# sanweiliti/RoHM

Hardware: NVIDIA H100
Metric: denoised motion clips/sec (145-frame, 1000-step PoseNet p_sample_loop) (higher is better)
Workload: dtype f32 (fp16 hi/lo error-compensated tensor-core GEMMs)

## Files before the change

### rohm_b200/csrc/graph.cu

```cuda
#include <algorithm>

#include "graph.cuh"

namespace rohm {

cudaError_t KernelPatch::apply(cudaGraphExec_t exec, cudaGraphNode_t node, const cudaKernelNodeParams& captured) const {
  void* args[kMaxArgs];
  std::copy(captured.kernelParams, captured.kernelParams + nargs_, args);
  for (int i = 0; i < n_; ++i) args[slots_[i].index] = const_cast<unsigned char*>(slots_[i].bytes);
  cudaKernelNodeParams kp = captured;
  kp.kernelParams = args;
  return cudaGraphExecKernelNodeSetParams(exec, node, &kp);
}

ForwardGraphs::~ForwardGraphs() {
  if (capture_stream_) cudaStreamDestroy(capture_stream_);
}

int ForwardGraphs::run(rohm_ctx* ctx, int B, int T, StepKind step, bool eager, cudaStream_t st,
                       const std::function<int(cudaStream_t)>& launches, const std::vector<KernelPatch>& patches,
                       const std::vector<int>& lengths) {
  cudaStreamCaptureStatus cap = cudaStreamCaptureStatusNone;
  ROHM_CUDA(ctx, cudaStreamIsCapturing(st, &cap));
  if (eager || !enabled || cap != cudaStreamCaptureStatusNone) return launches(st);

  Entry* g = nullptr;
  for (Entry& e : graphs_)
// ... 55 lines not shown
```

### rohm_b200/csrc/graph.cuh

```cuda
#pragma once
#include <cstring>
#include <functional>
#include <memory>
#include <tuple>
#include <type_traits>
#include <vector>

#include "common.h"

namespace rohm {

template <size_t I, typename V>
struct Arg {
  V value;
};
template <size_t I, typename V>
Arg<I, V> arg(V value) {
  return {value};
}

class KernelPatch {
 public:
  template <typename... P, size_t... I, typename... V>
  KernelPatch(void (*kernel)(P...), Arg<I, V>... args)
// ... 12 lines not shown
  };
  template <typename T, typename V>
  void put(size_t index, const V& value) {
    static_assert(std::is_same<V, T>::value || (std::is_pointer<V>::value && std::is_convertible<V, T>::value),
                  "KernelPatch: the value's type is not the kernel parameter's");
    static_assert(sizeof(T) <= sizeof(Slot::bytes), "KernelPatch: parameter wider than a slot");
    const T v = value;
    slots_[n_].index = index;
    std::memcpy(slots_[n_].bytes, &v, sizeof v);
    ++n_;
  }
  const void* func_;
  int nargs_;
  Slot slots_[kMaxPatched];
  int n_ = 0;
};

enum StepKind : int { kNoStep = 0, kStepSingleStream = 1, kStepPerClip = 2 };

class ForwardGraphs {
 public:
  static constexpr size_t kMaxGraphs = 8;
  bool enabled = true;

  ForwardGraphs() = default;
  ForwardGraphs(const ForwardGraphs&) = delete;
  ForwardGraphs& operator=(const ForwardGraphs&) = delete;
  ~ForwardGraphs();

  int run(rohm_ctx* ctx, int B, int T, StepKind step, bool eager, cudaStream_t st,
// ... 64 lines not shown
```

### rohm_b200/csrc/posenet.cu

```cuda
#include <cmath>
#include <cstdlib>
#include <cstring>
#include <new>

#include "attention.cuh"
#include "common.h"
#include "gemm.cuh"
#include "graph.cuh"
#include "ptx.cuh"

namespace rohm {
namespace {


__device__ __forceinline__ void clip_rows(const int* clip_off, int b, int S, int T, int64_t& row0, int& frames) {
  if (clip_off != nullptr) {
    row0 = clip_off[b];
    frames = clip_off[b + 1] - clip_off[b] - 1;
  } else {
    row0 = static_cast<int64_t>(b) * S;
    frames = T;
  }
}

// ... 176 lines not shown
      l.x = y.x - h.x, l.y = y.y - h.y, l.z = y.z - h.z, l.w = y.w - h.w;
      oh[lane + 32 * i] = h;
      ol[lane + 32 * i] = l;
    }
  }
}

}

struct PoseNetLayerDev {
  PackedWeight qkv, proj, ff1, ff2;
  float *qkv_b, *proj_b, *ff1_b, *ff2_b, *n1_w, *n1_b, *n2_w, *n2_b;
  float *qkv_c = nullptr, *qkv_d = nullptr, *ff1_c = nullptr, *ff1_d = nullptr;
};

}

using namespace rohm;

struct rohm_posenet {
  rohm_ctx* ctx = nullptr;
  DevicePool pool;
  int D = 0, F = 0, L = 0, H = 0, C = 0, Cout = 0, traj = 0, pe_len = 0, passes = 3;
  int kind = kKindTf32;
  int max_batch = 0, max_frames = 0;
  int64_t max_rows = 0;
  int Kin_p = 0;
  PackedWeight w_in, w_cond, w_out;
  float *in_b = nullptr, *cond_b = nullptr, *out_b = nullptr, *pe = nullptr;
  float* time_table = nullptr;
// ... 1 lines not shown
  float *Ain_h = nullptr, *Ain_l = nullptr;
  float *X = nullptr, *Xh = nullptr, *Xl = nullptr, *Y = nullptr, *QKV = nullptr, *CTXh = nullptr, *CTXl = nullptr;
  float *Hh = nullptr, *Hl = nullptr, *condpe = nullptr, *OUT = nullptr;
  float* cond_traj = nullptr;
  int cond_B = -1, cond_T = -1;
  std::vector<int> lengths;
  std::vector<int> cond_lengths;
  int* clip_off = nullptr;
  int* clip_ids = nullptr;
  int packed_rows = 0, n_short = 0, short_tokens = 0, long_tokens = 0;
  int launches = 0;
  ForwardGraphs graphs;
  bool use_pdl = true;
  bool tc_attention = false;
  bool attn_maps = false;
  AttnWgmmaMaps attn_wg{};
  AttnArgs attn{};
  bool fused_ln = false;
  float2* stats1 = nullptr;
  float2* stats2 = nullptr;
  float *out_c = nullptr, *out_d = nullptr;
  bool profiling = false;
  std::vector<cudaEvent_t> prof_events;
  std::vector<int> prof_cat;
  GemmParams g_in{}, g_cond{}, g_out{};
  std::vector<GemmParams> g_qkv, g_proj, g_ff1, g_ff2;
};

enum ProfCat { kCatGemm = 0, kCatAttention = 1, kCatLayerNorm = 2, kCatOther = 3, kNumCats = 4 };

static void prof_begin(rohm_posenet* pn, int cat, cudaStream_t st) {
  if (!pn->profiling) return;
  cudaEvent_t a, b;
  cudaEventCreate(&a);
  cudaEventCreate(&b);
  pn->prof_events.push_back(a);
  pn->prof_events.push_back(b);
  pn->prof_cat.push_back(cat);
  cudaEventRecord(a, st);
}
static void prof_end(rohm_posenet* pn, cudaStream_t st) {
// ... 144 lines not shown
  const int f16 = pn->kind == kKindF16 ? 1 : 0;
  const bool pdl = pn->use_pdl && !pn->profiling;
  switch (pn->D) {
    case 128: launch_ln<128>(in, res, g, b, out, oh, ol, rows, st, f16, pdl); break;
    case 256: launch_ln<256>(in, res, g, b, out, oh, ol, rows, st, f16, pdl); break;
    case 512: launch_ln<512>(in, res, g, b, out, oh, ol, rows, st, f16, pdl); break;
    case 1024: launch_ln<1024>(in, res, g, b, out, oh, ol, rows, st, f16, pdl); break;
    default: return fail(pn->ctx, ROHM_ERR_INVALID, "unsupported d_model %d for LayerNorm", pn->D);
  }
  prof_end(pn, st);
  ROHM_CUDA(pn->ctx, cudaGetLastError());
  pn->launches++;
  return ROHM_OK;
}

static int run_attention(rohm_posenet* pn, int B, int S, cudaStream_t st) {
  if (!pn->lengths.empty()) {
    const int n_long = B - pn->n_short;
    for (int k = 0; k < 2; ++k) {
      AttnArgs a = pn->attn;
      a.clip_off = pn->clip_off;
      a.clip_ids = pn->clip_ids + (k == 0 ? 0 : pn->n_short);
      a.B = k == 0 ? pn->n_short : n_long;
      a.S = k == 0 ? pn->short_tokens : pn->long_tokens;
      if (a.B == 0) continue;
      prof_begin(pn, kCatAttention, st);
      const cudaError_t e = launch_attention(a, k == 0 ? kAttnWgmma : kAttnWgmmaStream, &pn->attn_wg, st,
                                             pn->use_pdl && !pn->profiling);
      prof_end(pn, st);
      ROHM_CUDA(pn->ctx, e);
      pn->launches++;
    }
    return ROHM_OK;
  }
  AttnArgs a = pn->attn;
  a.B = B, a.S = S;
  const bool maps = pn->attn_maps && (pn->tc_attention || S > kAttnWgmmaMaxTokens);
  prof_begin(pn, kCatAttention, st);
  const cudaError_t e = launch_attention(a, kAttnAuto, maps ? &pn->attn_wg : nullptr, st, pn->use_pdl && !pn->profiling);
  prof_end(pn, st);
  ROHM_CUDA(pn->ctx, e);
  pn->launches++;
  return ROHM_OK;
}

static int build_time_table(rohm_posenet* pn, const rohm_posenet_weights* w) {
  const int D = pn->D, R = pn->pe_len;
  const int64_t n = static_cast<int64_t>(R) * D;
  pn->time_table = pn->pool.floats(n);
  if (pn->time_table == nullptr) return fail(pn->ctx, ROHM_ERR_CUDA, "time table alloc failed");
  DevicePool tmp;
  PackedWeight w0, w2;
  float* pe_h = tmp.floats(n);
  float* pe_l = tmp.floats(n);
// ... 9 lines not shown
  ROHM_CUDA(pn->ctx, cudaGetLastError());
  GemmParams g1{}, g2{};
  if ((rc = setup_linear(pn, &g1, pe_h, pe_l, R, D, D, w0, w->t0_b)) != ROHM_OK) return rc;
  g1.act = kActSilu;
  g1.out_hi = h_h, g1.out_lo = h_l, g1.lds = D;
  g1.M = R;
  ROHM_CUDA(pn->ctx, launch_gemm(g1, R, D, w0.block_n, 3, 0));
  if ((rc = setup_linear(pn, &g2, h_h, h_l, R, D, D, w2, bias2)) != ROHM_OK) return rc;
  g2.out = pn->time_table, g2.ldo = D;
  g2.M = R;
  ROHM_CUDA(pn->ctx, launch_gemm(g2, R, D, w2.block_n, 3, 0));
  ROHM_CUDA(pn->ctx, cudaDeviceSynchronize());
  return ROHM_OK;
}

extern "C" int rohm_posenet_create(rohm_ctx* ctx, const rohm_posenet_weights* w, int max_batch, int max_frames,
                                   int precision, rohm_posenet** out) {
  if (ctx == nullptr) return ROHM_ERR_INVALID;
  rohm::DeviceGuard device_guard__(ctx);
  if (w == nullptr || out == nullptr || max_batch <= 0 || max_frames <= 0)
    return fail(ctx, ROHM_ERR_INVALID, "rohm_posenet_create: bad arguments");
  if (precision != ROHM_PRECISION_TF32X3 && precision != ROHM_PRECISION_TF32 && precision != ROHM_PRECISION_F16X2)
    return fail(ctx, ROHM_ERR_INVALID, "rohm_posenet_create: precision must be 3 (TF32x3), 2 (F16x2) or 1 (TF32)");
  if (w->d_model % 128 != 0 || w->d_model % w->num_heads != 0 || w->ff_size % 64 != 0)
    return fail(ctx, ROHM_ERR_INVALID, "rohm_posenet_create: d_model must be a multiple of 128, ff_size of 64");
  const int dh = w->d_model / w->num_heads;
  if (dh != 64 && dh != 128) return fail(ctx, ROHM_ERR_INVALID, "rohm_posenet_create: head dim must be 64 or 128");
  if (max_frames + 1 > w->pe_len)
    return fail(ctx, ROHM_ERR_INVALID, "rohm_posenet_create: %d frames need %d rows of the positional table, which has %d",
                max_frames, max_frames + 1, w->pe_len);
// ... 106 lines not shown
  pn->clip_off = static_cast<int*>(pn->pool.bytes(static_cast<int64_t>(max_batch + 1) * sizeof(int)));
  pn->clip_ids = static_cast<int*>(pn->pool.bytes(static_cast<int64_t>(max_batch) * sizeof(int)));
  if (pn->clip_off == nullptr || pn->clip_ids == nullptr) {
    const int rc = fail(ctx, ROHM_ERR_CUDA, "clip table alloc failed: %s", cudaGetErrorString(pn->pool.last_error()));
    delete pn;
    return rc;
  }

  TRY(setup_linear(pn, &pn->g_in, pn->Ain_h, pn->Ain_l, R, pn->C, pn->Kin_p, pn->w_in, pn->in_b));
  pn->g_in.residual = pn->condpe, pn->g_in.ldr = D;
  pn->g_in.out = pn->X, pn->g_in.ldo = D;
  pn->g_in.out_hi = pn->Xh, pn->g_in.out_lo = pn->Xl, pn->g_in.lds = D;
  TRY(setup_linear(pn, &pn->g_cond, pn->Ain_h, pn->Ain_l, R, pn->C, pn->Kin_p, pn->w_cond, pn->cond_b));
  pn->g_cond.residual = pn->condpe, pn->g_cond.ldr = D;
  pn->g_cond.out = pn->condpe, pn->g_cond.ldo = D;
  TRY(setup_linear(pn, &pn->g_out, pn->Xh, pn->Xl, R, D, D, pn->w_out, pn->out_b));
  pn->g_out.out = pn->OUT, pn->g_out.ldo = pn->Cout;
  if (pn->fused_ln && pn->L > 0)
    pn->g_out.a_stats = pn->stats2, pn->g_out.a_corr = pn->out_c, pn->g_out.bias = pn->out_d, pn->g_out.ln_eps = 1e-5f;
  pn->g_qkv.resize(pn->L), pn->g_proj.resize(pn->L), pn->g_ff1.resize(pn->L), pn->g_ff2.resize(pn->L);
  for (int l = 0; l < pn->L; ++l) {
    PoseNetLayerDev& d = pn->layers[l];
    TRY(setup_linear(pn, &pn->g_qkv[l], pn->Xh, pn->Xl, R, D, D, d.qkv, d.qkv_b));
    if (pn->kind == kKindF16) {
      pn->g_qkv[l].out_hi = pn->QKV;
      pn->g_qkv[l].out_lo = reinterpret_cast<__half*>(pn->QKV) + R * 3 * D;
      pn->g_qkv[l].lds = 3 * D;
    } else {
      pn->g_qkv[l].out = pn->QKV, pn->g_qkv[l].ldo = 3 * D;
    }
    TRY(setup_linear(pn, &pn->g_proj[l], pn->CTXh, pn->CTXl, R, D, D, d.proj, d.proj_b));
    pn->g_proj[l].out = pn->Y, pn->g_proj[l].ldo = D;
    auto producer = [&](GemmParams& g, float2* stats_out, const float2* res_stats, const float* res_gamma, const float* res_beta) {
      g.out = nullptr, g.ldo = 0;
      g.out_hi = pn->Xh, g.out_lo = pn->Xl, g.lds = D;
      g.stats_out = stats_out, g.res_stats = res_stats, g.res_gamma = res_gamma, g.res_beta = res_beta, g.ln_eps = 1e-5f;
    };
    auto consumer = [&](GemmParams& g, const float2* a_stats, const float* c, const float* dvec) {
      g.a_stats = a_stats, g.a_corr = c, g.bias = dvec, g.ln_eps = 1e-5f;
    };
    if (pn->fused_ln) {
      if (l > 0) consumer(pn->g_qkv[l], pn->stats2, d.qkv_c, d.qkv_d);
      producer(pn->g_proj[l], pn->stats1, l > 0 ? pn->stats2 : nullptr, l > 0 ? pn->layers[l - 1].n2_w : nullptr,
               l > 0 ? pn->layers[l - 1].n2_b : nullptr);
    }
    TRY(setup_linear(pn, &pn->g_ff1[l], pn->Xh, pn->Xl, R, D, D, d.ff1, d.ff1_b));
    pn->g_ff1[l].act = kActGelu;
    pn->g_ff1[l].out_hi = pn->Hh, pn->g_ff1[l].out_lo = pn->Hl, pn->g_ff1[l].lds = F;
    TRY(setup_linear(pn, &pn->g_ff2[l], pn->Hh, pn->Hl, R, F, F, d.ff2, d.ff2_b));
    pn->g_ff2[l].out = pn->Y, pn->g_ff2[l].ldo = D;
    if (pn->fused_ln) {
      consumer(pn->g_ff1[l], pn->stats1, d.ff1_c, d.ff1_d);
      producer(pn->g_ff2[l], pn->stats2, pn->stats1, d.n1_w, d.n1_b);
    }
    for (GemmParams* g : {&pn->g_qkv[l], &pn->g_proj[l], &pn->g_ff1[l], &pn->g_ff2[l]}) {
      if (gemm_enable_tma_store(g, R, pn->kind) != 0) {
        const int rc__ = fail(ctx, ROHM_ERR_CUDA, "cuTensorMapEncodeTiled (store map) failed");
        delete pn;
        return rc__;
      }
    }
  }
  if (gemm_enable_tma_store(&pn->g_out, R, pn->kind) != 0) {
    const int rc__ = fail(ctx, ROHM_ERR_CUDA, "cuTensorMapEncodeTiled (store map) failed");
    delete pn;
    return rc__;
  }
#undef TRY

  {
    cudaError_t ea = gemm_init_attributes();
    if (ea == cudaSuccess) ea = attention_init_attributes(max_frames + 1, dh);
    if (ea != cudaSuccess) {
      delete pn;
      return fail(ctx, ROHM_ERR_CUDA, "kernel attribute setup failed: %s", cudaGetErrorString(ea));
    }
  }
  pn->attn.qkv_hi = pn->QKV;
  pn->attn.qkv_lo = reinterpret_cast<const __half*>(pn->QKV) + R * 3 * D;
  pn->attn.rows = R;
  pn->attn.ctx_hi = pn->CTXh, pn->attn.ctx_lo = pn->CTXl;
  pn->attn.D = D, pn->attn.H = pn->H;
  pn->attn.scale = 1.0f / sqrtf(static_cast<float>(dh));
  pn->attn.kind = pn->kind;
  pn->attn_maps = pn->kind == kKindF16 && dh == 128;
  if (pn->attn_maps) {
    const int rcm = attention_wgmma_maps(&pn->attn_wg, pn->attn);
    if (rcm != 0) {
      delete pn;
      return fail(ctx, ROHM_ERR_CUDA, "cuTensorMapEncodeTiled (attention tiles) failed (%d)", rcm);
    }
  }
  const cudaError_t e = cudaDeviceSynchronize();
  if (e != cudaSuccess) {
    delete pn;
    return fail(ctx, ROHM_ERR_CUDA, "weight packing failed: %s", cudaGetErrorString(e));
  }
  *out = pn;
  return ROHM_OK;
}

extern "C" void rohm_posenet_destroy(rohm_posenet* pn) { delete pn; }

extern "C" int rohm_posenet_launches_per_forward(const rohm_posenet* pn) { return pn ? pn->launches : 0; }

static int check_lengths(rohm_posenet* pn, int B, int T, const char* fn) {
// ... 72 lines not shown
      const bool is_short = S <= kAttnWgmmaMaxTokens;
      if (is_short != (pass == 0)) continue;
      ids.push_back(b);
      if (is_short) ++n_short, short_tokens = S > short_tokens ? S : short_tokens;
      else long_tokens = S > long_tokens ? S : long_tokens;
    }
  ROHM_CUDA(ctx, cudaDeviceSynchronize());
  ROHM_CUDA(ctx, cudaMemcpy(pn->clip_off, off.data(), (B + 1) * sizeof(int), cudaMemcpyHostToDevice));
  ROHM_CUDA(ctx, cudaMemcpy(pn->clip_ids, ids.data(), B * sizeof(int), cudaMemcpyHostToDevice));
  pn->lengths = std::move(v);
  pn->packed_rows = off[B];
  pn->n_short = n_short, pn->short_tokens = short_tokens, pn->long_tokens = long_tokens;
  return ROHM_OK;
}

static int forward_launches(rohm_posenet* pn, const float* x_t, const int64_t* timesteps, float* out, int B, int T,
                            cudaStream_t st) {
  rohm_ctx* ctx = pn->ctx;
  rohm::DeviceGuard device_guard__(ctx);
  const int S = T + 1, D = pn->D;
  const bool packed = !pn->lengths.empty();
  const int* off = packed ? pn->clip_off : nullptr;
  const int rows = packed ? pn->packed_rows : B * S;
  pn->launches = 0;
  int rc;

  dim3 grid((T + 31) / 32, (pn->C + 31) / 32, B);
  prof_begin(pn, kCatOther, st);
  const bool pdl = pn->use_pdl && !pn->profiling;
  ROHM_CUDA(ctx, launch_chain(pack_tokens_kernel, grid, dim3(32, 8), 0, st, pdl, x_t, pn->Ain_h, pn->Ain_l, pn->C, T, S, pn->Kin_p,
                              pn->kind == kKindF16 ? 1 : 0, off));
  prof_end(pn, st);
  ROHM_CUDA(ctx, cudaGetLastError());
  pn->launches++;
  if ((rc = run_gemm(pn, pn->g_in, pn->w_in, rows, st)) != ROHM_OK) return rc;
  prof_begin(pn, kCatOther, st);
  ROHM_CUDA(ctx, launch_chain(time_token_gather_kernel, dim3(B), dim3(128), 0, st, pdl, timesteps, pn->time_table, pn->pe_len,
                              pn->X, pn->Xh, pn->Xl, S, D, pn->kind == kKindF16 ? 1 : 0, off));
  prof_end(pn, st);
  ROHM_CUDA(ctx, cudaGetLastError());
  pn->launches++;

  for (int l = 0; l < pn->L; ++l) {
    PoseNetLayerDev& d = pn->layers[l];
    if ((rc = run_gemm(pn, pn->g_qkv[l], d.qkv, rows, st)) != ROHM_OK) return rc;
    if ((rc = run_attention(pn, B, S, st)) != ROHM_OK) return rc;
    if ((rc = run_gemm(pn, pn->g_proj[l], d.proj, rows, st)) != ROHM_OK) return rc;
    if (!pn->fused_ln && (rc = run_ln(pn, pn->Y, pn->X, d.n1_w, d.n1_b, pn->X, pn->Xh, pn->Xl, rows, st)) != ROHM_OK) return rc;
    if ((rc = run_gemm(pn, pn->g_ff1[l], d.ff1, rows, st)) != ROHM_OK) return rc;
    if ((rc = run_gemm(pn, pn->g_ff2[l], d.ff2, rows, st)) != ROHM_OK) return rc;
    if (!pn->fused_ln && (rc = run_ln(pn, pn->Y, pn->X, d.n2_w, d.n2_b, pn->X, pn->Xh, pn->Xl, rows, st)) != ROHM_OK) return rc;
  }
  if ((rc = run_gemm(pn, pn->g_out, pn->w_out, rows, st)) != ROHM_OK) return rc;
  dim3 grid_o((T + 31) / 32, (pn->Cout + 31) / 32, B);
  prof_begin(pn, kCatOther, st);
  ROHM_CUDA(ctx, launch_chain(unpack_tokens_kernel, grid_o, dim3(32, 8), 0, st, pdl, pn->OUT, pn->cond_traj, out, pn->C, pn->Cout,
                              pn->traj, T, S, pn->Cout, off));
  prof_end(pn, st);
  ROHM_CUDA(ctx, cudaGetLastError());
  pn->launches++;
  return ROHM_OK;
}

extern "C" int rohm_posenet_forward(rohm_posenet* pn, const float* x_t, const int64_t* timesteps, float* out, int B,
                                    int T, void* stream);

extern "C" int rohm_posenet_profile(rohm_posenet* pn, const float* x_t, const int64_t* timesteps, float* out, int B,
                                    int T, void* stream, float* ms_by_category, int* launches_by_category) {
  if (pn == nullptr) return ROHM_ERR_INVALID;
  if (ms_by_category == nullptr || launches_by_category == nullptr)
    return fail(pn->ctx, ROHM_ERR_INVALID, "rohm_posenet_profile: null output");
  pn->profiling = true;
  pn->prof_events.clear();
  pn->prof_cat.clear();
  int rc = rohm_posenet_forward(pn, x_t, timesteps, out, B, T, stream);
  pn->profiling = false;
  cudaError_t e = cudaStreamSynchronize(static_cast<cudaStream_t>(stream));
  for (int c = 0; c < kNumCats; ++c) ms_by_category[c] = 0.0f, launches_by_category[c] = 0;
  for (size_t i = 0; i < pn->prof_cat.size(); ++i) {
    float ms = 0.0f;
    if (rc == ROHM_OK && e == cudaSuccess) cudaEventElapsedTime(&ms, pn->prof_events[2 * i], pn->prof_events[2 * i + 1]);
    ms_by_category[pn->prof_cat[i]] += ms;
    launches_by_category[pn->prof_cat[i]]++;
  }
  for (cudaEvent_t ev : pn->prof_events) cudaEventDestroy(ev);
  pn->prof_events.clear();
  pn->prof_cat.clear();
  if (rc != ROHM_OK) return rc;
  ROHM_CUDA(pn->ctx, e);
  return ROHM_OK;
}
// ... 59 lines not shown
  if (rc != ROHM_OK) return rc;
  return forward_or_step(pn, x_t, timesteps, x0_out, B, T, stream, nullptr, &step);
}

extern "C" int rohm_posenet_set_option(rohm_posenet* pn, int option, int value) {
  if (pn == nullptr) return ROHM_ERR_INVALID;
  if (option == 0) {
    pn->graphs.enabled = value != 0;
    return ROHM_OK;
  }
  if (option == 1) {
    if (pn->use_pdl != (value != 0)) pn->graphs.clear();
    pn->use_pdl = value != 0;
    return ROHM_OK;
  }
  return fail(pn->ctx, ROHM_ERR_INVALID, "rohm_posenet_set_option: unknown option %d", option);
}
```

### rohm_b200/csrc/trajnet.cu

```cuda
#include <cmath>
#include <memory>
#include <new>
#include <string>

#include "common.h"
#include "gemm.cuh"
#include "graph.cuh"
#include "groupnorm.cuh"
#include "ptx.cuh"

namespace rohm {
namespace {

__device__ __forceinline__ int packed_frames(const int* clip_off, int b, int T, int Tp) {
  return clip_off[b + 1] - clip_off[b] - (Tp - T);
}

template <bool kPacked>
__global__ void pack_rows_kernel(const float* __restrict__ x, float* __restrict__ hi, float* __restrict__ lo, int T,
                                 int Tp, int C, int ld, int64_t total, int f16, const int* __restrict__ clip_off) {
  const int64_t i = static_cast<int64_t>(blockIdx.x) * blockDim.x + threadIdx.x;
  if (i >= total) return;
  const int c = static_cast<int>(i % C);
  const int64_t bt = i / C;
// ... 217 lines not shown
  Conv cond_down[3];
  Rtb enc[4], mid_block[2], dec[4];
  Conv down[4], up_even[4], up_odd[4];
  Conv final_c, final_o;
  GroupNorm final_gn;
  Act f1;
  struct {
    Conv z0, zero[4], down[4], zero_mid;
    Rtb enc[4], mid_block[2];
  } ctl;
  Act scratchY[2], scratchRes[2], scratchA[2];
  float* scratchSplit[2] = {nullptr, nullptr};
  bool use_splitk = true;
  bool parallel = true;
  cudaStream_t side[3] = {nullptr, nullptr, nullptr};
  std::vector<cudaEvent_t> events;
  size_t ev_next = 0;
  int cond_B = -1;
  int launches = 0;
  ForwardGraphs graphs;
  std::vector<int> lengths;
  std::vector<int> cond_lengths;
  int* clip_off[kLevels] = {};
  unsigned char* row_mask[kLevels] = {};
  int packed_rows[kLevels] = {};
  bool use_pdl = true;
  size_t gn_budget = 0;
  size_t gn_smem_max = 0;
  bool batch_invariant = false;
  ~rohm_trajnet() {
    for (cudaStream_t q : side)
      if (q) cudaStreamDestroy(q);
    for (cudaEvent_t e : events) cudaEventDestroy(e);
  }
};

#define TRY(expr)                     \
  do {                                \
    const int rc__ = (expr);          \
    if (rc__ != ROHM_OK) return rc__; \
  } while (0)

namespace {

int64_t rows_of(const rohm_trajnet* tn, int level) { return static_cast<int64_t>(tn->max_batch) * tn->Tp[level]; }

constexpr int64_t kInvariantPlanRows = 64 * (144 + 32);

// ... 246 lines not shown
  if (tn->batch_invariant && !tn->lengths.empty() && cv.gn_cluster > 1) {
    size_t smem = 0;
    for (int len : tn->lengths) {
      const int Tc = len >> level;
      smem = std::max(smem, gn_slice_bytes(Tc, C, kGroups, gn_pick_cluster(Tc, C, kGroups, kGnClipBudget)));
    }
    ROHM_CUDA(tn->ctx, launch_gn_mish_clip_slices(a, B, cv.gn_cluster, smem, st, tn->use_pdl, tn->clip_off[level]));
  } else {
    ROHM_CUDA(tn->ctx, launch_gn_mish(a, B, cv.gn_cluster, st, tn->use_pdl,
                                      tn->lengths.empty() ? nullptr : tn->clip_off[level]));
  }
  tn->launches++;
  return ROHM_OK;
}

int order_after(rohm_trajnet* tn, cudaStream_t from, cudaStream_t to) {
  if (from == to) return ROHM_OK;
  if (tn->ev_next == tn->events.size()) {
    cudaEvent_t e = nullptr;
    ROHM_CUDA(tn->ctx, cudaEventCreateWithFlags(&e, cudaEventDisableTiming));
    tn->events.push_back(e);
  }
  cudaEvent_t e = tn->events[tn->ev_next++];
  ROHM_CUDA(tn->ctx, cudaEventRecord(e, from));
  ROHM_CUDA(tn->ctx, cudaStreamWaitEvent(to, e, 0));
  return ROHM_OK;
}

int run_rtb(rohm_trajnet* tn, Rtb& r, int B, cudaStream_t st, cudaStream_t side) {
  if (r.has_res) {
    TRY(order_after(tn, st, side));
    TRY(run_conv(tn, r.res, B, side));
  }
  TRY(run_conv(tn, r.c1, B, st));
  const float* tp = r.tp_off >= 0 ? tn->tp + r.tp_off : nullptr;
  TRY(run_gn(tn, r.c1, r.gn[0], B, tp, nullptr, nullptr, r.a1, st));
  TRY(run_conv(tn, r.c2, B, st));
  if (r.has_res) TRY(order_after(tn, side, st));
  return run_gn(tn, r.c2, r.gn[1], B, nullptr, r.residual, r.extra, r.out, st);
}

int trajnet_create(rohm_ctx* ctx, int n_params, const char* const* names, const float* const* ptrs, const int64_t* numels,
                   int time_dim, int cond_dim, int traj_feat_dim, int mid_dim, int trajcontrol, int control_cond_dim,
                   int max_batch, int frames, int precision, bool batch_invariant, rohm_trajnet** out) {
  if (ctx == nullptr) return ROHM_ERR_INVALID;
  rohm::DeviceGuard device_guard__(ctx);
  if (names == nullptr || ptrs == nullptr || numels == nullptr || out == nullptr || max_batch <= 0)
    return fail(ctx, ROHM_ERR_INVALID, "rohm_trajnet_create: bad arguments");
  if (frames <= 0 || frames % 16 != 0)
    return fail(ctx, ROHM_ERR_INVALID, "rohm_trajnet_create: frames (%d) must be a positive multiple of 16 (four "
                "stride-2 stages)", frames);
  if (mid_dim <= 0 || mid_dim % 256 != 0 || time_dim % 2 != 0 || time_dim > 64)
    return fail(ctx, ROHM_ERR_INVALID, "rohm_trajnet_create: mid_dim (%d) must be a positive multiple of 256 (the GroupNorm "
// ... 270 lines not shown
  return ROHM_OK;
}

static int trajnet_forward_launches(rohm_trajnet* tn, const float* x_t, const int64_t* time, float* out, int B,
                                    cudaStream_t st) {
  rohm_ctx* ctx = tn->ctx;
  rohm::DeviceGuard device_guard__(ctx);
  tn->launches = 0;
  TRY(trajnet_pack(tn, x_t, tn->xin, B, st));
  const int td = tn->time_dim;
  trajnet_time_kernel<<<dim3(B, 8), 256, sizeof(float) * 6 * td, st>>>(time, td, tn->w1, tn->b1, tn->w3, tn->b3, tn->wcat, tn->bcat,
                                                            tn->tp_total, tn->tp, tn->time_table, kTimeTableRows);
  ROHM_CUDA(ctx, cudaGetLastError());
  tn->launches++;

  tn->ev_next = 0;
  if (tn->parallel)
    for (cudaStream_t& q : tn->side)
      if (q == nullptr) ROHM_CUDA(ctx, cudaStreamCreateWithFlags(&q, cudaStreamNonBlocking));
  cudaStream_t sC = (tn->parallel && tn->control) ? tn->side[0] : st;
  cudaStream_t r0 = tn->parallel ? tn->side[1] : st;
  cudaStream_t r1 = tn->parallel ? tn->side[2] : sC;
  if (tn->control) {
    auto& ctl = tn->ctl;
    TRY(order_after(tn, st, sC));
    for (int l = 0; l < 4; ++l) {
      TRY(run_rtb(tn, ctl.enc[l], B, sC, r1));
      TRY(run_conv(tn, ctl.zero[l], B, sC));
      TRY(run_conv(tn, ctl.down[l], B, sC));
    }
    for (Rtb& r : ctl.mid_block) TRY(run_rtb(tn, r, B, sC, r1));
    TRY(run_conv(tn, ctl.zero_mid, B, sC));
  }

  for (int l = 0; l < 4; ++l) {
    TRY(run_rtb(tn, tn->enc[l], B, st, r0));
    TRY(run_conv(tn, tn->down[l], B, st));
  }
  TRY(run_rtb(tn, tn->mid_block[0], B, st, r0));
  if (tn->control) TRY(order_after(tn, sC, st));
  TRY(run_rtb(tn, tn->mid_block[1], B, st, r0));
  for (int l = 3; l >= 0; --l) {
    TRY(order_after(tn, st, r0));
    TRY(run_conv(tn, tn->up_odd[l], B, r0));
    TRY(run_conv(tn, tn->up_even[l], B, st));
    TRY(order_after(tn, r0, st));
    TRY(run_rtb(tn, tn->dec[l], B, st, r0));
  }
  TRY(run_conv(tn, tn->final_c, B, st));
  TRY(run_gn(tn, tn->final_c, tn->final_gn, B, nullptr, nullptr, nullptr, tn->f1, st));
  TRY(run_conv(tn, tn->final_o, B, st));
  const Act& o = tn->final_o.out;
  const int64_t total = static_cast<int64_t>(B) * tn->T * o.C;
  const bool packed = !tn->lengths.empty();
  (packed ? unpack_rows_kernel<true> : unpack_rows_kernel<false>)<<<static_cast<unsigned>((total + 255) / 256), 256, 0, st>>>(
      o.f32, out, tn->T, tn->Tp[0], o.C, o.ld, total, packed ? tn->clip_off[0] : nullptr);
  ROHM_CUDA(ctx, cudaGetLastError());
  tn->launches++;
  return ROHM_OK;
}

// ... 77 lines not shown
```

Before: 20.16.

## Split PoseNet batch into two clip groups run on parallel streams

When the QKV GEMM tile count exceeds the SM count, the batch is split at a tile-aligned clip boundary into two row groups. Each group gets its own GEMM and attention parameter chain and runs on its own stream, forked and joined with events, so one group's attention and layer-norm phases can overlap the other group's GEMMs. The event-ordering helper moves out of TrajNet into a shared BranchEvents class. The cost is a second stream, extra per-shape plans and tensor maps, and smaller GEMMs that may use tensor cores less efficiently.

```diff
diff --git a/rohm_b200/csrc/graph.cu b/rohm_b200/csrc/graph.cu
--- a/rohm_b200/csrc/graph.cu
+++ b/rohm_b200/csrc/graph.cu
@@ -11,6 +11,23 @@
   cudaKernelNodeParams kp = captured;
   kp.kernelParams = args;
   return cudaGraphExecKernelNodeSetParams(exec, node, &kp);
+}
+
+BranchEvents::~BranchEvents() {
+  for (cudaEvent_t e : events_) cudaEventDestroy(e);
+}
+
+int BranchEvents::order_after(rohm_ctx* ctx, cudaStream_t from, cudaStream_t to) {
+  if (from == to) return ROHM_OK;
+  if (next_ == events_.size()) {
+    cudaEvent_t e = nullptr;
+    ROHM_CUDA(ctx, cudaEventCreateWithFlags(&e, cudaEventDisableTiming));
+    events_.push_back(e);
+  }
+  cudaEvent_t e = events_[next_++];
+  ROHM_CUDA(ctx, cudaEventRecord(e, from));
+  ROHM_CUDA(ctx, cudaStreamWaitEvent(to, e, 0));
+  return ROHM_OK;
 }
 
 ForwardGraphs::~ForwardGraphs() {
diff --git a/rohm_b200/csrc/graph.cuh b/rohm_b200/csrc/graph.cuh
--- a/rohm_b200/csrc/graph.cuh
+++ b/rohm_b200/csrc/graph.cuh
@@ -50,6 +50,20 @@
   int nargs_;
   Slot slots_[kMaxPatched];
   int n_ = 0;
+};
+
+class BranchEvents {
+ public:
+  BranchEvents() = default;
+  BranchEvents(const BranchEvents&) = delete;
+  BranchEvents& operator=(const BranchEvents&) = delete;
+  ~BranchEvents();
+  void rewind() { next_ = 0; }
+  int order_after(rohm_ctx* ctx, cudaStream_t from, cudaStream_t to);
+
+ private:
+  std::vector<cudaEvent_t> events_;
+  size_t next_ = 0;
 };
 
 enum StepKind : int { kNoStep = 0, kStepSingleStream = 1, kStepPerClip = 2 };
diff --git a/rohm_b200/csrc/posenet.cu b/rohm_b200/csrc/posenet.cu
--- a/rohm_b200/csrc/posenet.cu
+++ b/rohm_b200/csrc/posenet.cu
@@ -1,6 +1,7 @@
 #include <cmath>
 #include <cstdlib>
 #include <cstring>
+#include <memory>
 #include <new>
 
 #include "attention.cuh"
@@ -214,6 +215,19 @@
   float *qkv_c = nullptr, *qkv_d = nullptr, *ff1_c = nullptr, *ff1_d = nullptr;
 };
 
+struct LayerChain {
+  int64_t row0 = 0, rows = 0;
+  std::vector<GemmParams> qkv, proj, ff1, ff2;
+  GemmParams out{};
+  AttnArgs attn{};
+  AttnWgmmaMaps attn_wg{};
+};
+
+struct GroupPlan {
+  int B = 0, T = 0, split = 0;
+  LayerChain chain[2];
+};
+
 }
 
 using namespace rohm;
@@ -245,8 +259,6 @@
   bool use_pdl = true;
   bool tc_attention = false;
   bool attn_maps = false;
-  AttnWgmmaMaps attn_wg{};
-  AttnArgs attn{};
   bool fused_ln = false;
   float2* stats1 = nullptr;
   float2* stats2 = nullptr;
@@ -254,8 +266,16 @@
   bool profiling = false;
   std::vector<cudaEvent_t> prof_events;
   std::vector<int> prof_cat;
-  GemmParams g_in{}, g_cond{}, g_out{};
-  std::vector<GemmParams> g_qkv, g_proj, g_ff1, g_ff2;
+  GemmParams g_in{}, g_cond{};
+  LayerChain whole;
+  std::vector<std::unique_ptr<GroupPlan>> plans;
+  cudaStream_t side = nullptr;
+  BranchEvents forks;
+  int num_sms = 0;
+  int groups = 0;
+  ~rohm_posenet() {
+    if (side) cudaStreamDestroy(side);
+  }
 };
 
 enum ProfCat { kCatGemm = 0, kCatAttention = 1, kCatLayerNorm = 2, kCatOther = 3, kNumCats = 4 };
@@ -430,18 +450,18 @@
   return ROHM_OK;
 }
 
-static int run_attention(rohm_posenet* pn, int B, int S, cudaStream_t st) {
+static int run_attention(rohm_posenet* pn, const LayerChain& c, int B, int S, cudaStream_t st) {
   if (!pn->lengths.empty()) {
     const int n_long = B - pn->n_short;
     for (int k = 0; k < 2; ++k) {
-      AttnArgs a = pn->attn;
+      AttnArgs a = c.attn;
       a.clip_off = pn->clip_off;
       a.clip_ids = pn->clip_ids + (k == 0 ? 0 : pn->n_short);
       a.B = k == 0 ? pn->n_short : n_long;
       a.S = k == 0 ? pn->short_tokens : pn->long_tokens;
       if (a.B == 0) continue;
       prof_begin(pn, kCatAttention, st);
-      const cudaError_t e = launch_attention(a, k == 0 ? kAttnWgmma : kAttnWgmmaStream, &pn->attn_wg, st,
+      const cudaError_t e = launch_attention(a, k == 0 ? kAttnWgmma : kAttnWgmmaStream, &c.attn_wg, st,
                                              pn->use_pdl && !pn->profiling);
       prof_end(pn, st);
       ROHM_CUDA(pn->ctx, e);
@@ -449,11 +469,11 @@
     }
     return ROHM_OK;
   }
-  AttnArgs a = pn->attn;
+  AttnArgs a = c.attn;
   a.B = B, a.S = S;
   const bool maps = pn->attn_maps && (pn->tc_attention || S > kAttnWgmmaMaxTokens);
   prof_begin(pn, kCatAttention, st);
-  const cudaError_t e = launch_attention(a, kAttnAuto, maps ? &pn->attn_wg : nullptr, st, pn->use_pdl && !pn->profiling);
+  const cudaError_t e = launch_attention(a, kAttnAuto, maps ? &c.attn_wg : nullptr, st, pn->use_pdl && !pn->profiling);
   prof_end(pn, st);
   ROHM_CUDA(pn->ctx, e);
   pn->launches++;
@@ -493,6 +513,71 @@
   return ROHM_OK;
 }
 
+static int build_chain(rohm_posenet* pn, int64_t row0, int64_t rows, LayerChain* c) {
+  const int D = pn->D, F = pn->F, eb = gemm_elem_bytes(pn->kind);
+  const int64_t R = pn->max_rows;
+  auto at = [&](void* base, int64_t ld, int bytes) { return reinterpret_cast<float*>(static_cast<char*>(base) + row0 * ld * bytes); };
+  float *Xh = at(pn->Xh, D, eb), *Xl = at(pn->Xl, D, eb), *CTXh = at(pn->CTXh, D, eb), *CTXl = at(pn->CTXl, D, eb);
+  float *Hh = at(pn->Hh, F, eb), *Hl = at(pn->Hl, F, eb), *Y = at(pn->Y, D, 4), *OUT = at(pn->OUT, pn->Cout, 4);
+  float* qkv_hi = at(pn->QKV, 3 * D, eb);
+  float* qkv_lo = at(reinterpret_cast<__half*>(pn->QKV) + R * 3 * D, 3 * D, eb);
+  float2* stats1 = pn->fused_ln ? pn->stats1 + row0 * 8 : nullptr;
+  float2* stats2 = pn->fused_ln ? pn->stats2 + row0 * 8 : nullptr;
+  c->row0 = row0, c->rows = rows;
+  int rc;
+  if ((rc = setup_linear(pn, &c->out, Xh, Xl, rows, D, D, pn->w_out, pn->out_b)) != ROHM_OK) return rc;
+  c->out.out = OUT, c->out.ldo = pn->Cout;
+  if (pn->fused_ln && pn->L > 0)
+    c->out.a_stats = stats2, c->out.a_corr = pn->out_c, c->out.bias = pn->out_d, c->out.ln_eps = 1e-5f;
+  c->qkv.resize(pn->L), c->proj.resize(pn->L), c->ff1.resize(pn->L), c->ff2.resize(pn->L);
+  for (int l = 0; l < pn->L; ++l) {
+    PoseNetLayerDev& d = pn->layers[l];
+    if ((rc = setup_linear(pn, &c->qkv[l], Xh, Xl, rows, D, D, d.qkv, d.qkv_b)) != ROHM_OK) return rc;
+    if (pn->kind == kKindF16) {
+      c->qkv[l].out_hi = qkv_hi, c->qkv[l].out_lo = qkv_lo, c->qkv[l].lds = 3 * D;
+    } else {
+      c->qkv[l].out = qkv_hi, c->qkv[l].ldo = 3 * D;
+    }
+    if ((rc = setup_linear(pn, &c->proj[l], CTXh, CTXl, rows, D, D, d.proj, d.proj_b)) != ROHM_OK) return rc;
+    c->proj[l].out = Y, c->proj[l].ldo = D;
+    auto producer = [&](GemmParams& g, float2* stats_out, const float2* res_stats, const float* res_gamma, const float* res_beta) {
+      g.out = nullptr, g.ldo = 0;
+      g.out_hi = Xh, g.out_lo = Xl, g.lds = D;
+      g.stats_out = stats_out, g.res_stats = res_stats, g.res_gamma = res_gamma, g.res_beta = res_beta, g.ln_eps = 1e-5f;
+    };
+    auto consumer = [&](GemmParams& g, const float2* a_stats, const float* cv, const float* dvec) {
+      g.a_stats = a_stats, g.a_corr = cv, g.bias = dvec, g.ln_eps = 1e-5f;
+    };
+    if (pn->fused_ln) {
+      if (l > 0) consumer(c->qkv[l], stats2, d.qkv_c, d.qkv_d);
+      producer(c->proj[l], stats1, l > 0 ? stats2 : nullptr, l > 0 ? pn->layers[l - 1].n2_w : nullptr,
+               l > 0 ? pn->layers[l - 1].n2_b : nullptr);
+    }
+    if ((rc = setup_linear(pn, &c->ff1[l], Xh, Xl, rows, D, D, d.ff1, d.ff1_b)) != ROHM_OK) return rc;
+    c->ff1[l].act = kActGelu;
+    c->ff1[l].out_hi = Hh, c->ff1[l].out_lo = Hl, c->ff1[l].lds = F;
+    if ((rc = setup_linear(pn, &c->ff2[l], Hh, Hl, rows, F, F, d.ff2, d.ff2_b)) != ROHM_OK) return rc;
+    c->ff2[l].out = Y, c->ff2[l].ldo = D;
+    if (pn->fused_ln) {
+      consumer(c->ff1[l], stats1, d.ff1_c, d.ff1_d);
+      producer(c->ff2[l], stats2, stats1, d.n1_w, d.n1_b);
+    }
+    for (GemmParams* g : {&c->qkv[l], &c->proj[l], &c->ff1[l], &c->ff2[l]})
+      if (gemm_enable_tma_store(g, rows, pn->kind) != 0) return fail(pn->ctx, ROHM_ERR_CUDA, "cuTensorMapEncodeTiled (store map) failed");
+  }
+  if (gemm_enable_tma_store(&c->out, rows, pn->kind) != 0)
+    return fail(pn->ctx, ROHM_ERR_CUDA, "cuTensorMapEncodeTiled (store map) failed");
+  AttnArgs& a = c->attn;
+  a.qkv_hi = qkv_hi, a.qkv_lo = qkv_lo, a.rows = rows;
+  a.ctx_hi = CTXh, a.ctx_lo = CTXl;
+  a.D = D, a.H = pn->H;
+  a.scale = 1.0f / sqrtf(static_cast<float>(D / pn->H));
+  a.kind = pn->kind;
+  if (pn->attn_maps && (rc = attention_wgmma_maps(&c->attn_wg, a)) != 0)
+    return fail(pn->ctx, ROHM_ERR_CUDA, "cuTensorMapEncodeTiled (attention tiles) failed (%d)", rc);
+  return ROHM_OK;
+}
+
 extern "C" int rohm_posenet_create(rohm_ctx* ctx, const rohm_posenet_weights* w, int max_batch, int max_frames,
                                    int precision, rohm_posenet** out) {
   if (ctx == nullptr) return ROHM_ERR_INVALID;
@@ -629,60 +714,6 @@
   TRY(setup_linear(pn, &pn->g_cond, pn->Ain_h, pn->Ain_l, R, pn->C, pn->Kin_p, pn->w_cond, pn->cond_b));
   pn->g_cond.residual = pn->condpe, pn->g_cond.ldr = D;
   pn->g_cond.out = pn->condpe, pn->g_cond.ldo = D;
-  TRY(setup_linear(pn, &pn->g_out, pn->Xh, pn->Xl, R, D, D, pn->w_out, pn->out_b));
-  pn->g_out.out = pn->OUT, pn->g_out.ldo = pn->Cout;
-  if (pn->fused_ln && pn->L > 0)
-    pn->g_out.a_stats = pn->stats2, pn->g_out.a_corr = pn->out_c, pn->g_out.bias = pn->out_d, pn->g_out.ln_eps = 1e-5f;
-  pn->g_qkv.resize(pn->L), pn->g_proj.resize(pn->L), pn->g_ff1.resize(pn->L), pn->g_ff2.resize(pn->L);
-  for (int l = 0; l < pn->L; ++l) {
-    PoseNetLayerDev& d = pn->layers[l];
-    TRY(setup_linear(pn, &pn->g_qkv[l], pn->Xh, pn->Xl, R, D, D, d.qkv, d.qkv_b));
-    if (pn->kind == kKindF16) {
-      pn->g_qkv[l].out_hi = pn->QKV;
-      pn->g_qkv[l].out_lo = reinterpret_cast<__half*>(pn->QKV) + R * 3 * D;
-      pn->g_qkv[l].lds = 3 * D;
-    } else {
-      pn->g_qkv[l].out = pn->QKV, pn->g_qkv[l].ldo = 3 * D;
-    }
-    TRY(setup_linear(pn, &pn->g_proj[l], pn->CTXh, pn->CTXl, R, D, D, d.proj, d.proj_b));
-    pn->g_proj[l].out = pn->Y, pn->g_proj[l].ldo = D;
-    auto producer = [&](GemmParams& g, float2* stats_out, const float2* res_stats, const float* res_gamma, const float* res_beta) {
-      g.out = nullptr, g.ldo = 0;
-      g.out_hi = pn->Xh, g.out_lo = pn->Xl, g.lds = D;
-      g.stats_out = stats_out, g.res_stats = res_stats, g.res_gamma = res_gamma, g.res_beta = res_beta, g.ln_eps = 1e-5f;
-    };
-    auto consumer = [&](GemmParams& g, const float2* a_stats, const float* c, const float* dvec) {
-      g.a_stats = a_stats, g.a_corr = c, g.bias = dvec, g.ln_eps = 1e-5f;
-    };
-    if (pn->fused_ln) {
-      if (l > 0) consumer(pn->g_qkv[l], pn->stats2, d.qkv_c, d.qkv_d);
-      producer(pn->g_proj[l], pn->stats1, l > 0 ? pn->stats2 : nullptr, l > 0 ? pn->layers[l - 1].n2_w : nullptr,
-               l > 0 ? pn->layers[l - 1].n2_b : nullptr);
-    }
-    TRY(setup_linear(pn, &pn->g_ff1[l], pn->Xh, pn->Xl, R, D, D, d.ff1, d.ff1_b));
-    pn->g_ff1[l].act = kActGelu;
-    pn->g_ff1[l].out_hi = pn->Hh, pn->g_ff1[l].out_lo = pn->Hl, pn->g_ff1[l].lds = F;
-    TRY(setup_linear(pn, &pn->g_ff2[l], pn->Hh, pn->Hl, R, F, F, d.ff2, d.ff2_b));
-    pn->g_ff2[l].out = pn->Y, pn->g_ff2[l].ldo = D;
-    if (pn->fused_ln) {
-      consumer(pn->g_ff1[l], pn->stats1, d.ff1_c, d.ff1_d);
-      producer(pn->g_ff2[l], pn->stats2, pn->stats1, d.n1_w, d.n1_b);
-    }
-    for (GemmParams* g : {&pn->g_qkv[l], &pn->g_proj[l], &pn->g_ff1[l], &pn->g_ff2[l]}) {
-      if (gemm_enable_tma_store(g, R, pn->kind) != 0) {
-        const int rc__ = fail(ctx, ROHM_ERR_CUDA, "cuTensorMapEncodeTiled (store map) failed");
-        delete pn;
-        return rc__;
-      }
-    }
-  }
-  if (gemm_enable_tma_store(&pn->g_out, R, pn->kind) != 0) {
-    const int rc__ = fail(ctx, ROHM_ERR_CUDA, "cuTensorMapEncodeTiled (store map) failed");
-    delete pn;
-    return rc__;
-  }
-#undef TRY
-
   {
     cudaError_t ea = gemm_init_attributes();
     if (ea == cudaSuccess) ea = attention_init_attributes(max_frames + 1, dh);
@@ -691,20 +722,14 @@
       return fail(ctx, ROHM_ERR_CUDA, "kernel attribute setup failed: %s", cudaGetErrorString(ea));
     }
   }
-  pn->attn.qkv_hi = pn->QKV;
-  pn->attn.qkv_lo = reinterpret_cast<const __half*>(pn->QKV) + R * 3 * D;
-  pn->attn.rows = R;
-  pn->attn.ctx_hi = pn->CTXh, pn->attn.ctx_lo = pn->CTXl;
-  pn->attn.D = D, pn->attn.H = pn->H;
-  pn->attn.scale = 1.0f / sqrtf(static_cast<float>(dh));
-  pn->attn.kind = pn->kind;
   pn->attn_maps = pn->kind == kKindF16 && dh == 128;
-  if (pn->attn_maps) {
-    const int rcm = attention_wgmma_maps(&pn->attn_wg, pn->attn);
-    if (rcm != 0) {
-      delete pn;
-      return fail(ctx, ROHM_ERR_CUDA, "cuTensorMapEncodeTiled (attention tiles) failed (%d)", rcm);
-    }
+  TRY(build_chain(pn, 0, R, &pn->whole));
+#undef TRY
+  int dev = 0;
+  if (cudaGetDevice(&dev) != cudaSuccess || cudaDeviceGetAttribute(&pn->num_sms, cudaDevAttrMultiProcessorCount, dev) != cudaSuccess ||
+      cudaStreamCreateWithFlags(&pn->side, cudaStreamNonBlocking) != cudaSuccess) {
+    delete pn;
+    return fail(ctx, ROHM_ERR_CUDA, "stream creation failed");
   }
   const cudaError_t e = cudaDeviceSynchronize();
   if (e != cudaSuccess) {
@@ -807,6 +832,64 @@
   return ROHM_OK;
 }
 
+static int run_layer(rohm_posenet* pn, LayerChain& c, int l, int B, int S, int rows, cudaStream_t st) {
+  PoseNetLayerDev& d = pn->layers[l];
+  int rc;
+  if ((rc = run_gemm(pn, c.qkv[l], d.qkv, rows, st)) != ROHM_OK) return rc;
+  if ((rc = run_attention(pn, c, B, S, st)) != ROHM_OK) return rc;
+  if ((rc = run_gemm(pn, c.proj[l], d.proj, rows, st)) != ROHM_OK) return rc;
+  const int64_t r0 = c.row0 * pn->D;
+  const int eb = gemm_elem_bytes(pn->kind);
+  float *X = pn->X + r0, *Y = pn->Y + r0;
+  float* Xh = reinterpret_cast<float*>(reinterpret_cast<char*>(pn->Xh) + r0 * eb);
+  float* Xl = reinterpret_cast<float*>(reinterpret_cast<char*>(pn->Xl) + r0 * eb);
+  if (!pn->fused_ln && (rc = run_ln(pn, Y, X, d.n1_w, d.n1_b, X, Xh, Xl, rows, st)) != ROHM_OK) return rc;
+  if ((rc = run_gemm(pn, c.ff1[l], d.ff1, rows, st)) != ROHM_OK) return rc;
+  if ((rc = run_gemm(pn, c.ff2[l], d.ff2, rows, st)) != ROHM_OK) return rc;
+  if (!pn->fused_ln && (rc = run_ln(pn, Y, X, d.n2_w, d.n2_b, X, Xh, Xl, rows, st)) != ROHM_OK) return rc;
+  return ROHM_OK;
+}
+
+static int split_point(int B, int S) {
+  int best = 1;
+  int64_t best_tiles = -1;
+  for (int k = 1; k < B; ++k) {
+    const int64_t tiles = (static_cast<int64_t>(k) * S + kGemmBlockM - 1) / kGemmBlockM +
+                          (static_cast<int64_t>(B - k) * S + kGemmBlockM - 1) / kGemmBlockM;
+    if (best_tiles < 0 || tiles < best_tiles || (tiles == best_tiles && std::abs(2 * k - B) < std::abs(2 * best - B)))
+      best = k, best_tiles = tiles;
+  }
+  return best;
+}
+
+static bool use_groups(const rohm_posenet* pn, int B, int S) {
+  const int64_t row_tiles = (static_cast<int64_t>(B) * S + kGemmBlockM - 1) / kGemmBlockM;
+  const int64_t col_tiles = pn->L > 0 ? pn->layers[0].qkv.Np / pn->layers[0].qkv.block_n : 0;
+  return row_tiles * col_tiles > pn->num_sms;
+}
+
+static int group_plan(rohm_posenet* pn, int B, int T, GroupPlan** plan) {
+  *plan = nullptr;
+  const int S = T + 1;
+  const bool split = pn->groups == 2 || (pn->groups == 0 && use_groups(pn, B, S));
+  if (B < 2 || !pn->lengths.empty() || pn->profiling || !split) return ROHM_OK;
+  for (const auto& p : pn->plans)
+    if (p->B == B && p->T == T) {
+      *plan = p.get();
+      return ROHM_OK;
+    }
+  std::unique_ptr<GroupPlan> p(new (std::nothrow) GroupPlan());
+  if (p == nullptr) return fail(pn->ctx, ROHM_ERR_INVALID, "out of host memory");
+  p->B = B, p->T = T, p->split = split_point(B, S);
+  int rc = build_chain(pn, 0, static_cast<int64_t>(p->split) * S, &p->chain[0]);
+  if (rc == ROHM_OK) rc = build_chain(pn, static_cast<int64_t>(p->split) * S, static_cast<int64_t>(B - p->split) * S, &p->chain[1]);
+  if (rc != ROHM_OK) return rc;
+  if (pn->plans.size() >= ForwardGraphs::kMaxGraphs) pn->plans.erase(pn->plans.begin());
+  pn->plans.push_back(std::move(p));
+  *plan = pn->plans.back().get();
+  return ROHM_OK;
+}
+
 static int forward_launches(rohm_posenet* pn, const float* x_t, const int64_t* timesteps, float* out, int B, int T,
                             cudaStream_t st) {
   rohm_ctx* ctx = pn->ctx;
@@ -834,17 +917,26 @@
   ROHM_CUDA(ctx, cudaGetLastError());
   pn->launches++;
 
-  for (int l = 0; l < pn->L; ++l) {
-    PoseNetLayerDev& d = pn->layers[l];
-    if ((rc = run_gemm(pn, pn->g_qkv[l], d.qkv, rows, st)) != ROHM_OK) return rc;
-    if ((rc = run_attention(pn, B, S, st)) != ROHM_OK) return rc;
-    if ((rc = run_gemm(pn, pn->g_proj[l], d.proj, rows, st)) != ROHM_OK) return rc;
-    if (!pn->fused_ln && (rc = run_ln(pn, pn->Y, pn->X, d.n1_w, d.n1_b, pn->X, pn->Xh, pn->Xl, rows, st)) != ROHM_OK) return rc;
-    if ((rc = run_gemm(pn, pn->g_ff1[l], d.ff1, rows, st)) != ROHM_OK) return rc;
-    if ((rc = run_gemm(pn, pn->g_ff2[l], d.ff2, rows, st)) != ROHM_OK) return rc;
-    if (!pn->fused_ln && (rc = run_ln(pn, pn->Y, pn->X, d.n2_w, d.n2_b, pn->X, pn->Xh, pn->Xl, rows, st)) != ROHM_OK) return rc;
-  }
-  if ((rc = run_gemm(pn, pn->g_out, pn->w_out, rows, st)) != ROHM_OK) return rc;
+  GroupPlan* plan = nullptr;
+  if ((rc = group_plan(pn, B, T, &plan)) != ROHM_OK) return rc;
+  if (plan == nullptr) {
+    for (int l = 0; l < pn->L; ++l)
+      if ((rc = run_layer(pn, pn->whole, l, B, S, rows, st)) != ROHM_OK) return rc;
+    if ((rc = run_gemm(pn, pn->whole.out, pn->w_out, rows, st)) != ROHM_OK) return rc;
+  } else {
+    const cudaStream_t gst[2] = {st, pn->side};
+    const int clips[2] = {plan->split, B - plan->split};
+    pn->forks.rewind();
+    if ((rc = pn->forks.order_after(ctx, st, pn->side)) != ROHM_OK) return rc;
+    for (int l = 0; l < pn->L; ++l)
+      for (int g = 0; g < 2; ++g)
+        if ((rc = run_layer(pn, plan->chain[g], l, clips[g], S, static_cast<int>(plan->chain[g].rows), gst[g])) != ROHM_OK)
+          return rc;
+    for (int g = 0; g < 2; ++g)
+      if ((rc = run_gemm(pn, plan->chain[g].out, pn->w_out, static_cast<int>(plan->chain[g].rows), gst[g])) != ROHM_OK)
+        return rc;
+    if ((rc = pn->forks.order_after(ctx, pn->side, st)) != ROHM_OK) return rc;
+  }
   dim3 grid_o((T + 31) / 32, (pn->Cout + 31) / 32, B);
   prof_begin(pn, kCatOther, st);
   ROHM_CUDA(ctx, launch_chain(unpack_tokens_kernel, grid_o, dim3(32, 8), 0, st, pdl, pn->OUT, pn->cond_traj, out, pn->C, pn->Cout,
@@ -866,8 +958,10 @@
   pn->profiling = true;
   pn->prof_events.clear();
   pn->prof_cat.clear();
+  const int launches = pn->launches;
   int rc = rohm_posenet_forward(pn, x_t, timesteps, out, B, T, stream);
   pn->profiling = false;
+  if (launches > 0) pn->launches = launches;
   cudaError_t e = cudaStreamSynchronize(static_cast<cudaStream_t>(stream));
   for (int c = 0; c < kNumCats; ++c) ms_by_category[c] = 0.0f, launches_by_category[c] = 0;
   for (size_t i = 0; i < pn->prof_cat.size(); ++i) {
@@ -957,5 +1051,11 @@
     pn->use_pdl = value != 0;
     return ROHM_OK;
   }
+  if (option == 2) {
+    if (value < 0 || value > 2) return fail(pn->ctx, ROHM_ERR_INVALID, "rohm_posenet_set_option(2): value must be 0, 1 or 2");
+    if (pn->groups != value) pn->graphs.clear();
+    pn->groups = value;
+    return ROHM_OK;
+  }
   return fail(pn->ctx, ROHM_ERR_INVALID, "rohm_posenet_set_option: unknown option %d", option);
 }
diff --git a/rohm_b200/csrc/trajnet.cu b/rohm_b200/csrc/trajnet.cu
--- a/rohm_b200/csrc/trajnet.cu
+++ b/rohm_b200/csrc/trajnet.cu
@@ -255,8 +255,7 @@
   bool use_splitk = true;
   bool parallel = true;
   cudaStream_t side[3] = {nullptr, nullptr, nullptr};
-  std::vector<cudaEvent_t> events;
-  size_t ev_next = 0;
+  BranchEvents events;
   int cond_B = -1;
   int launches = 0;
   ForwardGraphs graphs;
@@ -272,7 +271,6 @@
   ~rohm_trajnet() {
     for (cudaStream_t q : side)
       if (q) cudaStreamDestroy(q);
-    for (cudaEvent_t e : events) cudaEventDestroy(e);
   }
 };
 
@@ -549,29 +547,16 @@
   return ROHM_OK;
 }
 
-int order_after(rohm_trajnet* tn, cudaStream_t from, cudaStream_t to) {
-  if (from == to) return ROHM_OK;
-  if (tn->ev_next == tn->events.size()) {
-    cudaEvent_t e = nullptr;
-    ROHM_CUDA(tn->ctx, cudaEventCreateWithFlags(&e, cudaEventDisableTiming));
-    tn->events.push_back(e);
-  }
-  cudaEvent_t e = tn->events[tn->ev_next++];
-  ROHM_CUDA(tn->ctx, cudaEventRecord(e, from));
-  ROHM_CUDA(tn->ctx, cudaStreamWaitEvent(to, e, 0));
-  return ROHM_OK;
-}
-
 int run_rtb(rohm_trajnet* tn, Rtb& r, int B, cudaStream_t st, cudaStream_t side) {
   if (r.has_res) {
-    TRY(order_after(tn, st, side));
+    TRY(tn->events.order_after(tn->ctx, st, side));
     TRY(run_conv(tn, r.res, B, side));
   }
   TRY(run_conv(tn, r.c1, B, st));
   const float* tp = r.tp_off >= 0 ? tn->tp + r.tp_off : nullptr;
   TRY(run_gn(tn, r.c1, r.gn[0], B, tp, nullptr, nullptr, r.a1, st));
   TRY(run_conv(tn, r.c2, B, st));
-  if (r.has_res) TRY(order_after(tn, side, st));
+  if (r.has_res) TRY(tn->events.order_after(tn->ctx, side, st));
   return run_gn(tn, r.c2, r.gn[1], B, nullptr, r.residual, r.extra, r.out, st);
 }
 
@@ -872,7 +857,7 @@
   ROHM_CUDA(ctx, cudaGetLastError());
   tn->launches++;
 
-  tn->ev_next = 0;
+  tn->events.rewind();
   if (tn->parallel)
     for (cudaStream_t& q : tn->side)
       if (q == nullptr) ROHM_CUDA(ctx, cudaStreamCreateWithFlags(&q, cudaStreamNonBlocking));
@@ -881,7 +866,7 @@
   cudaStream_t r1 = tn->parallel ? tn->side[2] : sC;
   if (tn->control) {
     auto& ctl = tn->ctl;
-    TRY(order_after(tn, st, sC));
+    TRY(tn->events.order_after(tn->ctx, st, sC));
     for (int l = 0; l < 4; ++l) {
       TRY(run_rtb(tn, ctl.enc[l], B, sC, r1));
       TRY(run_conv(tn, ctl.zero[l], B, sC));
@@ -896,13 +881,13 @@
     TRY(run_conv(tn, tn->down[l], B, st));
   }
   TRY(run_rtb(tn, tn->mid_block[0], B, st, r0));
-  if (tn->control) TRY(order_after(tn, sC, st));
+  if (tn->control) TRY(tn->events.order_after(tn->ctx, sC, st));
   TRY(run_rtb(tn, tn->mid_block[1], B, st, r0));
   for (int l = 3; l >= 0; --l) {
-    TRY(order_after(tn, st, r0));
+    TRY(tn->events.order_after(tn->ctx, st, r0));
     TRY(run_conv(tn, tn->up_odd[l], B, r0));
     TRY(run_conv(tn, tn->up_even[l], B, st));
-    TRY(order_after(tn, r0, st));
+    TRY(tn->events.order_after(tn->ctx, r0, st));
     TRY(run_rtb(tn, tn->dec[l], B, st, r0));
   }
   TRY(run_conv(tn, tn->final_c, B, st));
```

After: 21.68, median of 6. 7.5% higher.
